# TorchIO-project/torchio

Measured on NVIDIA H100. Metric: augmented voxels/sec on 256^3 fp32 Compose pipeline, higher is better.
Workload: dtype f32

## Files before the change

### torchio_b200/csrc/fused_intensity.cu

```cuda
#include "common.cuh"
#include "mt19937_layout.h"
#include "mt19937_normal.cuh"
#include "tma.cuh"

namespace tio {

__device__ __forceinline__ float rician(float x, float n1, float n2) {
  float s = __fadd_rn(x, n1);
  return sqrtf(__fadd_rn(__fmul_rn(s, s), __fmul_rn(n2, n2)));
}


__device__ __forceinline__ uint4 philox4x32_10(uint4 ctr, uint2 key) {
  const uint32_t M0 = 0xD2511F53u, M1 = 0xCD9E8D57u, W0 = 0x9E3779B9u, W1 = 0xBB67AE85u;
#pragma unroll
  for (int r = 0; r < 7; ++r) {
    uint32_t hi0 = __umulhi(M0, ctr.x), lo0 = M0 * ctr.x;
    uint32_t hi1 = __umulhi(M1, ctr.z), lo1 = M1 * ctr.z;
    ctr = make_uint4(hi1 ^ ctr.y ^ key.x, lo1, hi0 ^ ctr.w ^ key.y, lo0);
    key.x += W0;
    key.y += W1;
  }
  return ctr;
}
// ... 508 lines not shown
          float b1 = lerp2(lk[v].l0, p1[lj.i1 * bi.sk + lk[v].i0], lk[v].l1, p1[lj.i1 * bi.sk + lk[v].i1]);
          r_hi[v] = lerp2(lj.l0, b0, lj.l1, b1);
        }
        cur0 = li.i0; cur1 = li.i1;
      }
#pragma unroll
      for (int v = 0; v < V; ++v) {
        float f = expf(lerp2(li.l0, r_lo[v], li.l1, r_hi[v]));
        out[v] = bi.divide ? __fdiv_rn(out[v], f) : __fmul_rn(out[v], f);
      }
    }
  };

  auto finish = [&](int i, float* v) {
    const int64_t o = ((int64_t)i * J + j) * K + k;
    if (noise_on) {
      const int64_t flat = (int64_t)bc * n + o;
      float z1[V], z2[V];
      if (nz.mode == 1) {
        if (V == 4) {
          float4 t = __ldcs((const float4*)(nz.z + flat));
          z1[0] = t.x; z1[1] = t.y; z1[2] = t.z; z1[3] = t.w;
          if (nz.rician) {
            float4 u = __ldcs((const float4*)(nz.z2 + flat));
            z2[0] = u.x; z2[1] = u.y; z2[2] = u.z; z2[3] = u.w;
          }
        } else {
          z1[0] = nz.z[flat];
          if (nz.rician) z2[0] = nz.z2[flat];
        }
      } else {
        const uint2 key = make_uint2((uint32_t)nz.philox_seed, (uint32_t)(nz.philox_seed >> 32));
        const uint64_t gidx = (uint64_t)(flat / V);
        uint4 rr = philox4x32_10(make_uint4((uint32_t)gidx, (uint32_t)(gidx >> 32), 0u, 0x5eedu), key);
        float nn[4];
        box_muller(rr.x, rr.y, nn[0], nn[1]);
        box_muller(rr.z, rr.w, nn[2], nn[3]);
#pragma unroll
        for (int q = 0; q < V; ++q) z1[q] = nn[q];
        if (nz.rician) {
          uint4 r2 = philox4x32_10(make_uint4((uint32_t)gidx, (uint32_t)(gidx >> 32), 1u, 0x5eedu), key);
          box_muller(r2.x, r2.y, nn[0], nn[1]);
          box_muller(r2.z, r2.w, nn[2], nn[3]);
#pragma unroll
          for (int q = 0; q < V; ++q) z2[q] = nn[q];
        }
      }
#pragma unroll
      for (int q = 0; q < V; ++q) {
        float n1 = __fadd_rn(mu, __fmul_rn(sd, z1[q]));
        if (nz.rician) v[q] = rician(v[q], n1, __fadd_rn(mu, __fmul_rn(sd, z2[q])));
        else v[q] = __fadd_rn(v[q], n1);
      }
    }
    if (gamma) {
#pragma unroll
      for (int q = 0; q < V; ++q) v[q] = signed_pow(v[q], gam);
    }
    if (V == 4) *(float4*)(y + o) = make_float4(v[0], v[1], v[2], v[3]);
    else y[o] = v[0];
  };

  if (r == 0) {
    for (int i = 0; i < I; ++i) {
      float v[V];
      load_plane(i, v);
      finish(i, v);
    }
    return;
  }

  float* mine = ring + tid * V;
  const int slot_stride = 256 * V;
  auto put = [&](int pos, const float* v) {
    int s = pos % W; if (s < 0) s += W;
    if (V == 4) *(float4*)(mine + s * slot_stride) = make_float4(v[0], v[1], v[2], v[3]);
    else mine[s * slot_stride] = v[0];
  };
  float first[V];
  load_plane(0, first);
  for (int p = -r; p <= 0; ++p) put(p, first);
  float last[V];
#pragma unroll
  for (int q = 0; q < V; ++q) last[q] = first[q];
  for (int p = 1; p < I + r; ++p) {
    if (p < I) load_plane(p, last);
    put(p, last);
    const int o = p - r;
    if (o < 0) continue;
    float acc[V];
#pragma unroll
    for (int q = 0; q < V; ++q) acc[q] = 0.0f;
    int s = (o - r) % W; if (s < 0) s += W;
    for (int t = 0; t < W; ++t) {
      const float tp = tapi[R - r + t];
      if (V == 4) {
        float4 w4 = *(const float4*)(mine + s * slot_stride);
        acc[0] = __fmaf_rn(tp, w4.x, acc[0]); acc[1] = __fmaf_rn(tp, w4.y, acc[1]);
        acc[2] = __fmaf_rn(tp, w4.z, acc[2]); acc[3] = __fmaf_rn(tp, w4.w, acc[3]);
      } else {
        acc[0] = __fmaf_rn(tp, mine[s * slot_stride], acc[0]);
      }
      if (++s == W) s = 0;
    }
    finish(o, acc);
  }
}

constexpr int M6_PF = 8;

template <bool HAS_BIAS, bool EPI, int BAR>
__device__ __forceinline__ void march6_tile(float* smem, const int tid, const int k, const int j, const int bc,
                                            const float* __restrict__ src, float* __restrict__ dst, int B,
                                            int C, int I, int J, int K, const BlurArgs& bl, const BiasArgs& bi,
                                            const NoiseArgs& nz, const float* __restrict__ gamma) {
  constexpr int W = 2 * F_R + 1;
  const int b = bc / C;
  const int64_t n = (int64_t)I * J * K;
  const float* x = src + (int64_t)bc * n;
  float* y = dst + (int64_t)bc * n;

  const int r = bl.taps ? bl.radius[0 * B + b] : 0;
  float* tapi = smem;
  float* g = smem + 16;
  const int ns = HAS_BIAS ? bi.si * bi.sj * bi.sk : 0;
  const bool bias_on = HAS_BIAS && !(bi.identity && bi.identity[b]);
  if (tid < W) {
    const int off = tid - F_R;
    tapi[tid] = (r > 0 && off >= -r && off <= r) ? bl.taps[((int64_t)0 * B + b) * (2 * bl.R + 1) + bl.R + off] : 0.0f;
  }
  if (bias_on) {
    const float* gs = bi.coarse + (int64_t)bc * ns;
    for (int t = tid; t < ns; t += 256) g[t] = gs[t];
  }
  if (BAR == 0) __syncthreads();
  else asm volatile("bar.sync %0, 256;" ::"n"(BAR) : "memory");
  if (k >= K || j >= J) return;

  const bool noise_on = EPI && nz.mode != 0 && (!nz.keep || nz.keep[b]);
  const float mu = (EPI && nz.mode) ? nz.mean[b] : 0.0f, sd = (EPI && nz.mode) ? nz.std[b] : 0.0f;
  const float gam = (EPI && gamma) ? gamma[b] : 1.0f;
  const int gamma_mode = !(EPI && gamma) || gam == 1.0f ? 0 : (gam > 0.0f ? 1 : 2);

  LerpAxis lj, lk[4];
  int o00[4], o01[4], o10[4], o11[4];
  int cur0 = -1, cur1 = -1;
  float r_lo[4], r_hi[4];
  if (bias_on) {
    lj = lerp_axis(bi.sc_j, bi.sj, j);
#pragma unroll
    for (int v = 0; v < 4; ++v) {
      lk[v] = lerp_axis(bi.sc_k, bi.sk, k + v);
      o00[v] = lj.i0 * bi.sk + lk[v].i0; o01[v] = lj.i0 * bi.sk + lk[v].i1;
      o10[v] = lj.i1 * bi.sk + lk[v].i0; o11[v] = lj.i1 * bi.sk + lk[v].i1;
    }
  }
  const int col = j * K + k;
  const int plane = J * K;

  float4* fifo = reinterpret_cast<float4*>(g + ((ns + 3) / 4) * 4) + tid;
  auto fifo_issue = [&](int pl) {
    if (pl < I) {
      const uint32_t sa = (uint32_t)__cvta_generic_to_shared(fifo + (pl & (M6_PF - 1)) * 256);
      asm volatile("cp.async.cg.shared.global [%0], [%1], 16;" ::"r"(sa), "l"(x + (int64_t)pl * plane + col) : "memory");
    }
    asm volatile("cp.async.commit_group;" ::: "memory");
  };
#pragma unroll
  for (int pl = 0; pl < M6_PF - 1; ++pl) fifo_issue(pl);

  auto load_plane = [&](int i, float* out) {
    fifo_issue(i + M6_PF - 1);
    asm volatile("cp.async.wait_group %0;" ::"n"(M6_PF - 1) : "memory");
    const float4 t = fifo[(i & (M6_PF - 1)) * 256];
    out[0] = t.x; out[1] = t.y; out[2] = t.z; out[3] = t.w;
    if (bias_on) {
      const LerpAxis li = lerp_axis(bi.sc_i, bi.si, i);
      if (li.i0 != cur0 || li.i1 != cur1) {
        const float* p0 = g + (li.i0 * bi.sj) * bi.sk;
        const float* p1 = g + (li.i1 * bi.sj) * bi.sk;
#pragma unroll
        for (int v = 0; v < 4; ++v) {
          const float a0 = lerp2(lk[v].l0, p0[o00[v]], lk[v].l1, p0[o01[v]]);
          const float a1 = lerp2(lk[v].l0, p0[o10[v]], lk[v].l1, p0[o11[v]]);
          r_lo[v] = lerp2(lj.l0, a0, lj.l1, a1);
          const float b0 = lerp2(lk[v].l0, p1[o00[v]], lk[v].l1, p1[o01[v]]);
          const float b1 = lerp2(lk[v].l0, p1[o10[v]], lk[v].l1, p1[o11[v]]);
          r_hi[v] = lerp2(lj.l0, b0, lj.l1, b1);
        }
        cur0 = li.i0; cur1 = li.i1;
      }
#pragma unroll
      for (int v = 0; v < 4; ++v) {
        const float f = expf(lerp2(li.l0, r_lo[v], li.l1, r_hi[v]));
        out[v] = bi.divide ? __fdiv_rn(out[v], f) : __fmul_rn(out[v], f);
      }
    }
  };

  auto finish = [&](int i, float* v) {
    const int64_t o = (int64_t)i * plane + col;
    if (EPI) {
      if (noise_on) {
        const int64_t flat = (int64_t)bc * n + o;
        float z1[4], z2[4];
        if (nz.mode == 1) {
          const float4 t = __ldcs((const float4*)(nz.z + flat));
          z1[0] = t.x; z1[1] = t.y; z1[2] = t.z; z1[3] = t.w;
          if (nz.rician) {
            const float4 u = __ldcs((const float4*)(nz.z2 + flat));
            z2[0] = u.x; z2[1] = u.y; z2[2] = u.z; z2[3] = u.w;
          }
        } else {
          const uint2 key = make_uint2((uint32_t)nz.philox_seed, (uint32_t)(nz.philox_seed >> 32));
          const uint64_t gidx = (uint64_t)(flat / 4);
          uint4 rr = philox4x32_10(make_uint4((uint32_t)gidx, (uint32_t)(gidx >> 32), 0u, 0x5eedu), key);
          box_muller(rr.x, rr.y, z1[0], z1[1]);
          box_muller(rr.z, rr.w, z1[2], z1[3]);
          if (nz.rician) {
            uint4 r2 = philox4x32_10(make_uint4((uint32_t)gidx, (uint32_t)(gidx >> 32), 1u, 0x5eedu), key);
            box_muller(r2.x, r2.y, z2[0], z2[1]);
            box_muller(r2.z, r2.w, z2[2], z2[3]);
          }
        }
#pragma unroll
        for (int q = 0; q < 4; ++q) {
          const float n1 = __fadd_rn(mu, __fmul_rn(sd, z1[q]));
          if (nz.rician) v[q] = rician(v[q], n1, __fadd_rn(mu, __fmul_rn(sd, z2[q])));
          else v[q] = __fadd_rn(v[q], n1);
        }
      }
      if (gamma_mode == 1) {
#pragma unroll
        for (int q = 0; q < 4; ++q) v[q] = signed_pow_pos(v[q], gam);
      } else if (gamma_mode == 2) {
#pragma unroll
        for (int q = 0; q < 4; ++q) v[q] = signed_pow(v[q], gam);
      }
    }
    *(float4*)(y + o) = make_float4(v[0], v[1], v[2], v[3]);
  };

  if (r == 0) {
    for (int i = 0; i < I; ++i) {
      float v[4];
      load_plane(i, v);
      finish(i, v);
    }
    return;
  }

  float tp[W];
#pragma unroll
  for (int t = 0; t < W; ++t) tp[t] = tapi[t];
  float ring[W][4];
  {
    float first[4];
    load_plane(0, first);
#pragma unroll
    for (int sl = 0; sl < W; ++sl)
#pragma unroll
      for (int q = 0; q < 4; ++q) ring[sl][q] = first[q];
  }
  for (int base = 0; base < I + F_R; base += W) {
#pragma unroll
    for (int ph = 0; ph < W; ++ph) {
      const int p = base + ph;
      if (p >= I + F_R) break;
      if (p > 0 && p < I) load_plane(p, ring[ph]);
      else if (p >= I) {
#pragma unroll
        for (int q = 0; q < 4; ++q) ring[ph][q] = ring[(ph + W - 1) % W][q];
      }
      const int o = p - F_R;
      if (o >= 0) {
        float acc[4] = {0.0f, 0.0f, 0.0f, 0.0f};
#pragma unroll
        for (int t = 0; t < W; ++t) {
          if (t < F_R - r || t > F_R + r) continue;
          const int sl = (ph + 1 + t) % W;
#pragma unroll
          for (int q = 0; q < 4; ++q) acc[q] = __fmaf_rn(tp[t], ring[sl][q], acc[q]);
        }
        finish(o, acc);
      }
    }
  }
}

template <bool HAS_BIAS, bool EPI>
__global__ void __launch_bounds__(256, EPI ? 1 : 2)
march6_kernel(const float* __restrict__ src, float* __restrict__ dst, int B, int C, int I, int J,
              int K, BlurArgs bl, BiasArgs bi, NoiseArgs nz, const float* __restrict__ gamma) {
  extern __shared__ __align__(16) float smem[];
  march6_tile<HAS_BIAS, EPI, 0>(smem, threadIdx.y * blockDim.x + threadIdx.x,
                                (blockIdx.x * blockDim.x + threadIdx.x) * 4,
                                blockIdx.y * blockDim.y + threadIdx.y, blockIdx.z, src, dst, B, C, I, J, K,
                                bl, bi, nz, gamma);
}

constexpr int P1N_MARCH_THREADS = 256;
constexpr int P1N_THREADS = P1N_MARCH_THREADS + 5 * 128;
constexpr int P1N_BAR_SEGMENT = 6, P1N_BAR_MARCH = 7;
constexpr int P1N_RING_FLOATS = MT_RING * MT_N + 4;

template <bool HAS_BIAS>
__global__ void __launch_bounds__(P1N_THREADS, 1)
pass1_normals_kernel(const float* __restrict__ src, float* __restrict__ dst, int B, int C, int I, int J,
                     int K, BlurArgs bl, BiasArgs bi, unsigned int* __restrict__ tile_counter,
                     const uint32_t* __restrict__ states, int q_lo, int q_hi, unsigned long long L,
                     unsigned long long offset, unsigned long long n, float* __restrict__ z) {
  extern __shared__ __align__(16) float smem[];
  if (threadIdx.x < P1N_MARCH_THREADS) {
    asm volatile("setmaxnreg.inc.sync.aligned.u32 152;");
    const int tid = threadIdx.x;
    volatile int* next_tile = reinterpret_cast<int*>(smem + MT_RING * MT_N);
    const int kb_n = (K + 255) / 256, jb_n = (J + 3) / 4;
    const int tiles = kb_n * jb_n * B * C;
    for (;;) {
      if (tid == 0) *next_tile = (int)atomicAdd(tile_counter, 1u);
      asm volatile("bar.sync %0, 256;" ::"n"(P1N_BAR_MARCH) : "memory");
      const int tile = *next_tile;
      if (tile >= tiles) break;
      const int kb = tile % kb_n, jb = (tile / kb_n) % jb_n, bc = tile / (kb_n * jb_n);
      march6_tile<HAS_BIAS, false, P1N_BAR_MARCH>(smem + P1N_RING_FLOATS, tid, (kb * 64 + (tid & 63)) * 4,
                                                  jb * 4 + (tid >> 6), bc, src, dst, B, C, I, J, K, bl, bi,
                                                  NoiseArgs{}, nullptr);
    }
  } else {
    asm volatile("setmaxnreg.dec.sync.aligned.u32 40;");
    const int tid = threadIdx.x - P1N_MARCH_THREADS;
    if (tid >= MT_THREADS) return;
    for (int q = q_lo + blockIdx.x; q < q_hi; q += gridDim.x) {
      mt_normal_segment(reinterpret_cast<uint32_t*>(smem), tid, states, q, L, offset, n, z);
      mt_bar_sync<P1N_BAR_SEGMENT, MT_THREADS>();
    }
  }
}

constexpr int WIDE_RMAX = 6143;

template <bool HAS_EPI>
__global__ void __launch_bounds__(256)
axis_kernel(const float* __restrict__ src, float* __restrict__ dst, int B, int C, int I, int J,
            int K, int axis, BlurArgs bl, NoiseArgs nz, const float* __restrict__ gamma) {
  extern __shared__ float taps_s[];
  const int bc = blockIdx.y;
  const int b = bc / C;
  const int tid = threadIdx.x;
  const int64_t n = (int64_t)I * J * K;
  const int r = bl.radius[axis * B + b];
  for (int t = tid; t < 2 * r + 1; t += 256)
    taps_s[t] = bl.taps[((int64_t)axis * B + b) * (2 * bl.R + 1) + bl.R - r + t];
  __syncthreads();
  const int64_t e = (int64_t)blockIdx.x * 256 + tid;
  if (e >= n) return;
  const int L = axis == 0 ? I : (axis == 1 ? J : K);
  const int64_t s = axis == 0 ? (int64_t)J * K : (axis == 1 ? K : 1);
  const int pos = (int)((e / s) % L);
  const float* x = src + (int64_t)bc * n + (e - pos * s);
  float acc;
  if (r == 0) {
    acc = x[pos * s];
  } else {
    acc = 0.0f;
    for (int t = 0; t <= 2 * r; ++t) {
      const int q = min(max(pos - r + t, 0), L - 1);
      acc = __fmaf_rn(taps_s[t], __ldg(x + q * s), acc);
    }
  }
  const int64_t flat = (int64_t)bc * n + e;
  if (HAS_EPI) {
    if (nz.mode != 0 && (!nz.keep || nz.keep[b])) {
      const float mu = nz.mean[b], sd = nz.std[b];
      float z1, z2 = 0.0f;
      if (nz.mode == 1) {
        z1 = nz.z[flat];
        if (nz.rician) z2 = nz.z2[flat];
      } else {
        const uint2 key = make_uint2((uint32_t)nz.philox_seed, (uint32_t)(nz.philox_seed >> 32));
        float unused;
        uint4 rr = philox4x32_10(make_uint4((uint32_t)flat, (uint32_t)((uint64_t)flat >> 32), 0u, 0x77ffu), key);
        box_muller(rr.x, rr.y, z1, unused);
        if (nz.rician) box_muller(rr.z, rr.w, z2, unused);
      }
      const float n1 = __fadd_rn(mu, __fmul_rn(sd, z1));
      acc = nz.rician ? rician(acc, n1, __fadd_rn(mu, __fmul_rn(sd, z2))) : __fadd_rn(acc, n1);
    }
    if (gamma) acc = signed_pow(acc, gamma[b]);
  }
  dst[flat] = acc;
}

static inline bool aligned16f(const void* p) { return ((uintptr_t)p & 15) == 0; }

static float up_scale(int n_in, int n_out) {
  if (n_in == n_out) return 1.0f;
  return n_out > 1 ? (float)(n_in - 1) / (float)(n_out - 1) : 0.0f;
}

template <int RMAX>
static int launch_jk(const float* src, float* dst, int B, int C, int I, int J, int K,
                     const BlurArgs& bl, const NoiseArgs& nz, const float* gamma, cudaStream_t st) {
  constexpr int ROWS = A_TJ + 2 * RMAX, COLS = A_TK + 2 * RMAX, PITCH = (COLS + 3) / 4 * 4 + 4;
  const size_t smem = (size_t)(ROWS * PITCH + ROWS * A_TK + 2 * (2 * RMAX + 1)) * sizeof(float);
  const int tiles_i = (I + A_PLANES - 1) / A_PLANES;
  dim3 grid((K + A_TK - 1) / A_TK, (J + A_TJ - 1) / A_TJ, B * C * tiles_i);
  if (nz.mode != 0 || gamma) {
    if (smem > 48 * 1024)
      cudaFuncSetAttribute(jk_kernel<RMAX, true>, cudaFuncAttributeMaxDynamicSharedMemorySize, (int)smem);
    jk_kernel<RMAX, true><<<grid, 256, smem, st>>>(src, dst, B, C, I, J, K, bl, nz, gamma);
  } else {
    if (smem > 48 * 1024)
      cudaFuncSetAttribute(jk_kernel<RMAX, false>, cudaFuncAttributeMaxDynamicSharedMemorySize, (int)smem);
    jk_kernel<RMAX, false><<<grid, 256, smem, st>>>(src, dst, B, C, I, J, K, bl, nz, gamma);
  }
  launched();
  return 0;
}

static int launch_march(const float* cur, float* out, int B, int C, int I, int J, int K,
                        const BiasArgs& bi, const BlurArgs& ib, const NoiseArgs& nz1,
                        const float* gamma1, cudaStream_t st, const char* who) {
  {
    const bool vec = (K % 4 == 0) && aligned16f(cur) && aligned16f(out) &&
                     (nz1.mode != 1 || (aligned16f(nz1.z) && (!nz1.z2 || aligned16f(nz1.z2))));
    const int V = vec ? 4 : 1;
    dim3 block(64, 4);
    dim3 grid((K + 64 * V - 1) / (64 * V), (J + 3) / 4, B * C);
    TIO_CHECK_ARG(grid.y <= 65535, "%s: J too large", who);
    const int R = ib.taps ? ib.R : 0;
    const int ns = bi.coarse ? bi.si * bi.sj * bi.sk : 0;
    const size_t smem = ((size_t)((2 * R + 1 + 3) / 4 * 4) + (size_t)((ns + 3) / 4 * 4) +
                         (ib.taps ? (size_t)(2 * R + 1) * 256 * V : 0)) * sizeof(float);
#define TIO_LAUNCH_MARCH(VV, BB)                                                              \
  do {                                                                                        \
    if (smem > 48 * 1024)                                                                     \
      cudaFuncSetAttribute(march_kernel<VV, BB>, cudaFuncAttributeMaxDynamicSharedMemorySize, \
                           (int)smem);                                                        \
    march_kernel<VV, BB><<<grid, block, smem, st>>>(cur, out, B, C, I, J, K, ib, bi, nz1, gamma1); \
    launched();                                                                               \
  } while (0)
    if (vec && R <= F_R) {
      const size_t smem6 = (size_t)(16 + (ns + 3) / 4 * 4) * sizeof(float) + (size_t)M6_PF * 256 * 16;
#define TIO_LAUNCH_MARCH6(BB, EE)                                                              \
  do {                                                                                         \
    if (smem6 > 48 * 1024)                                                                     \
      cudaFuncSetAttribute(march6_kernel<BB, EE>, cudaFuncAttributeMaxDynamicSharedMemorySize, \
                           (int)smem6);                                                        \
    march6_kernel<BB, EE><<<grid, block, smem6, st>>>(cur, out, B, C, I, J, K, ib, bi, nz1, gamma1); \
    launched();                                                                                \
  } while (0)
      const bool epi = nz1.mode != 0 || gamma1 != nullptr;
      if (bi.coarse) { if (epi) TIO_LAUNCH_MARCH6(true, true); else TIO_LAUNCH_MARCH6(true, false); }
      else { if (epi) TIO_LAUNCH_MARCH6(false, true); else TIO_LAUNCH_MARCH6(false, false); }
#undef TIO_LAUNCH_MARCH6
    } else if (vec) { if (bi.coarse) TIO_LAUNCH_MARCH(4, true); else TIO_LAUNCH_MARCH(4, false); }
    else { if (bi.coarse) TIO_LAUNCH_MARCH(1, true); else TIO_LAUNCH_MARCH(1, false); }
#undef TIO_LAUNCH_MARCH
  }
  return 0;
}

static int wide_impl(const float* src, float* dst, float* scratch, int B, int C, int I, int J,
                     int K, const BiasArgs& bi, const BlurArgs& bl, int axes_mask,
                     const NoiseArgs& nz, const float* gamma, cudaStream_t st, const char* who) {
  TIO_CHECK_ARG(bl.R <= WIDE_RMAX, "%s: blur radius R=%d > %d unsupported", who, bl.R, WIDE_RMAX);
  int axes[3], na = 0;
  for (int a : {0, 2, 1})
    if (axes_mask & (1 << a)) axes[na++] = a;
  const int steps = na + (bi.coarse ? 1 : 0);
  TIO_CHECK_ARG(src != dst && (steps < 2 || (scratch && scratch != src && scratch != dst)),
                "%s: blur radius R=%d > 16 needs src != dst and a scratch buffer", who, bl.R);
  const int64_t n = (int64_t)I * J * K;
  TIO_CHECK_ARG((n + 255) / 256 <= 0x7fffffff, "%s: volume too large", who);
  const float* cur = src;
  int left = steps;
  auto next_out = [&]() { return (--left % 2 == 0) ? dst : scratch; };
  if (bi.coarse) {
    BlurArgs none = bl;
    none.taps = nullptr;
    float* out = next_out();
    if (launch_march(cur, out, B, C, I, J, K, bi, none, NoiseArgs{}, nullptr, st, who)) return 1;
    cur = out;
  }
  const size_t smem = (size_t)(2 * bl.R + 1) * sizeof(float);
  dim3 grid((unsigned)((n + 255) / 256), B * C);
  for (int s = 0; s < na; ++s) {
    float* out = next_out();
    if (s == na - 1 && (nz.mode != 0 || gamma))
      axis_kernel<true><<<grid, 256, smem, st>>>(cur, out, B, C, I, J, K, axes[s], bl, nz, gamma);
    else
      axis_kernel<false><<<grid, 256, smem, st>>>(cur, out, B, C, I, J, K, axes[s], bl, nz, gamma);
    launched();
    cur = out;
  }
  TIO_CHECK_LAUNCH();
  return 0;
}

static int fused_impl(const float* src, float* dst, float* scratch, int B, int C, int I, int J,
                      int K, BiasArgs bi, BlurArgs bl, int axes_mask, NoiseArgs nz,
                      const float* gamma, cudaStream_t st, const char* who) {
  TIO_CHECK_ARG(src && dst, "%s: null src/dst", who);
  TIO_CHECK_ARG(B > 0 && C > 0 && I > 0 && J > 0 && K > 0, "%s: bad shape", who);
  TIO_CHECK_ARG((int64_t)B * C <= 65535, "%s: B*C must be <= 65535", who);
  if (!bl.taps) axes_mask = 0;
  TIO_CHECK_ARG(!bl.taps || (bl.radius && bl.R >= 0), "%s: blur radius table missing or R=%d < 0", who, bl.R);
  if (bi.coarse) {
    bi.sc_i = up_scale(bi.si, I); bi.sc_j = up_scale(bi.sj, J); bi.sc_k = up_scale(bi.sk, K);
    TIO_CHECK_ARG((size_t)bi.si * bi.sj * bi.sk * 4 <= 64 * 1024, "%s: coarse bias grid too large", who);
  }
  if (axes_mask != 0 && bl.R > 16)
    return wide_impl(src, dst, scratch, B, C, I, J, K, bi, bl, axes_mask, nz, gamma, st, who);
  const bool need_jk = (axes_mask & 6) != 0;
  const bool need_i = (axes_mask & 1) != 0;
  const bool need_march = !need_jk || need_i || bi.coarse != nullptr;
  TIO_CHECK_ARG(!need_jk || src != dst, "%s: blur along J/K needs src != dst", who);
  TIO_CHECK_ARG(!(need_jk && need_march) || (scratch && scratch != src && scratch != dst),
                "%s: blur along J/K after bias or blur along I needs a scratch buffer", who);
  TIO_CHECK_ARG(!((axes_mask & 1) && src == dst && !need_jk), "%s: blur along I needs src != dst", who);
  const float* cur = src;
  if (need_jk) {
    const int64_t tiles = (int64_t)B * C * ((I + A_PLANES - 1) / A_PLANES);
    TIO_CHECK_ARG(tiles <= 65535, "%s: batch too large for the blur grid", who);
  }
  if (need_march) {
    BlurArgs ib = bl;
    if (!need_i) ib.taps = nullptr;
    float* out = need_jk ? scratch : dst;
    if (launch_march(cur, out, B, C, I, J, K, bi, ib, need_jk ? NoiseArgs{} : nz,
                     need_jk ? nullptr : gamma, st, who))
      return 1;
    cur = out;
  }
  if (need_jk) {
    const bool tma_ok = bl.R <= F_R && (K % 4 == 0) && aligned16f(cur) && (int64_t)B * C * I < (1ll << 31);
    EncodeTiledFn encode = tma_ok ? encode_tiled_fn() : nullptr;
    CUtensorMap tm;
    bool have_map = false;
    if (encode) {
      const cuuint64_t gdim[3] = {(cuuint64_t)K, (cuuint64_t)J, (cuuint64_t)B * C * I};
      const cuuint64_t gstride[2] = {(cuuint64_t)K * 4, (cuuint64_t)J * K * 4};
      const cuuint32_t bdim[3] = {(cuuint32_t)F_COLS, (cuuint32_t)F_ROWS, 1};
      const cuuint32_t estr[3] = {1, 1, 1};
      have_map = encode(&tm, CU_TENSOR_MAP_DATA_TYPE_FLOAT32, 3, const_cast<float*>(cur), gdim, gstride,
                        bdim, estr, CU_TENSOR_MAP_INTERLEAVE_NONE, CU_TENSOR_MAP_SWIZZLE_NONE,
                        CU_TENSOR_MAP_L2_PROMOTION_L2_128B, CU_TENSOR_MAP_FLOAT_OOB_FILL_NONE) == CUDA_SUCCESS;
    }
    if (have_map) {
      const int tiles_i = (I + A_PLANES - 1) / A_PLANES;
      dim3 grid((K + A_TK - 1) / A_TK, (J + A_TJ - 1) / A_TJ, B * C * tiles_i);
      if (nz.mode != 0 || gamma) {
        cudaFuncSetAttribute(jk6_kernel<true>, cudaFuncAttributeMaxDynamicSharedMemorySize, (int)F_SMEM);
        jk6_kernel<true><<<grid, 256, F_SMEM, st>>>(tm, dst, B, C, I, J, K, bl, nz, gamma);
      } else {
        cudaFuncSetAttribute(jk6_kernel<false>, cudaFuncAttributeMaxDynamicSharedMemorySize, (int)F_SMEM);
        jk6_kernel<false><<<grid, 256, F_SMEM, st>>>(tm, dst, B, C, I, J, K, bl, nz, gamma);
      }
      launched();
    } else if (bl.R <= F_R) {
      launch_jk<6>(cur, dst, B, C, I, J, K, bl, nz, gamma, st);
    } else {
      launch_jk<16>(cur, dst, B, C, I, J, K, bl, nz, gamma, st);
    }
  }
  TIO_CHECK_LAUNCH();
  return 0;
}

}

using namespace tio;

extern "C" int tio_blur(const float* src, float* dst, float* scratch, int B, int C, int I, int J,
                        int K, const float* taps, const int32_t* radius, int R, int axes_mask,
                        const uint8_t* identity, void* stream) {
  (void)identity;
  TIO_CHECK_ARG(taps && radius, "tio_blur: null taps/radius");
  TIO_CHECK_ARG(src != dst, "tio_blur: src and dst must not alias");
  BiasArgs bi{};
  BlurArgs bl{taps, radius, R};
  NoiseArgs nz{};
  return fused_impl(src, dst, scratch, B, C, I, J, K, bi, bl, axes_mask & 7, nz, nullptr,
                    (cudaStream_t)stream, "tio_blur");
}

extern "C" int tio_intensity_fused(const float* src, float* dst, float* scratch, int B, int C,
                                   int I, int J, int K, const float* coarse, int si, int sj,
                                   int sk, const uint8_t* bias_identity, int bias_divide,
                                   const float* taps, const int32_t* radius, int R,
                                   int axes_mask, const float* mean, const float* std,
                                   const uint8_t* keep, const float* z, const float* z2,
                                   uint64_t philox_seed, int noise_mode, int rician_flag,
                                   const float* gamma, void* stream) {
  BiasArgs bi{};
  bi.coarse = coarse; bi.identity = bias_identity; bi.si = si; bi.sj = sj; bi.sk = sk;
  bi.divide = bias_divide;
  BlurArgs bl{taps, radius, R};
  NoiseArgs nz{};
  nz.mode = noise_mode;
  TIO_CHECK_ARG(noise_mode >= 0 && noise_mode <= 2, "tio_intensity_fused: bad noise_mode");
  if (noise_mode) {
    TIO_CHECK_ARG(mean && std, "tio_intensity_fused: noise needs mean/std");
    TIO_CHECK_ARG(noise_mode != 1 || (z && (!rician_flag || z2)), "tio_intensity_fused: normals missing");
    nz.mean = mean; nz.std = std; nz.keep = keep; nz.z = z; nz.z2 = z2;
    nz.philox_seed = philox_seed; nz.rician = rician_flag;
  }
  return fused_impl(src, dst, scratch, B, C, I, J, K, bi, bl, taps ? (axes_mask & 7) : 0, nz,
                    gamma, (cudaStream_t)stream, "tio_intensity_fused");
}

extern "C" size_t tio_intensity_pass1_with_normals_workspace_bytes(uint64_t offset, uint64_t n) {
  return tio_randn_mt19937_workspace_bytes(offset, n) + 16;
}

extern "C" int tio_intensity_pass1_with_normals(const float* src, float* dst, int B, int C, int I, int J,
                                                int K, const float* coarse, int si, int sj, int sk,
                                                const uint8_t* bias_identity, int bias_divide,
                                                const float* taps, const int32_t* radius, int R,
                                                int axes_mask, uint64_t seed, uint64_t offset, uint64_t n,
                                                float* z, const void* table, void* workspace,
                                                size_t workspace_bytes, void* stream) {
  const char* who = "tio_intensity_pass1_with_normals";
  TIO_CHECK_ARG(src && dst && z, "%s: null src/dst/z", who);
  TIO_CHECK_ARG(src != dst, "%s: src and dst must not alias", who);
  TIO_CHECK_ARG(B > 0 && C > 0 && I > 0 && J > 0 && K > 0, "%s: bad shape", who);
  const bool need_i = taps && (axes_mask & 1);
  TIO_CHECK_ARG(!need_i || (radius && R >= 0 && R <= F_R), "%s: needs a radius table and R <= %d, got R=%d", who,
                F_R, R);
  TIO_CHECK_ARG(K % 4 == 0 && aligned16f(src) && aligned16f(dst) && aligned16f(z),
                "%s: needs K %% 4 == 0 and 16-byte aligned src, dst and z", who);
  const int64_t tiles = (int64_t)((K + 255) / 256) * ((J + 3) / 4) * B * C;
  TIO_CHECK_ARG(tiles < (1ll << 31) - (1 << 20), "%s: batch too large", who);
  BiasArgs bi{};
  bi.coarse = coarse; bi.identity = bias_identity; bi.si = si; bi.sj = sj; bi.sk = sk;
  bi.divide = bias_divide;
  if (coarse) {
    bi.sc_i = up_scale(si, I); bi.sc_j = up_scale(sj, J); bi.sc_k = up_scale(sk, K);
    TIO_CHECK_ARG(si > 0 && sj > 0 && sk > 0 && (size_t)si * sj * sk * 4 <= 64 * 1024,
                  "%s: coarse bias grid empty or too large", who);
  }
  BlurArgs bl{need_i ? taps : nullptr, radius, R};
  TIO_CHECK_ARG(workspace_bytes >= tio_intensity_pass1_with_normals_workspace_bytes(offset, n),
                "%s: workspace too small", who);
  cudaStream_t st = (cudaStream_t)stream;
  int q_lo, q_hi;
  const size_t states_bytes = tio_randn_mt19937_workspace_bytes(offset, n);
  if (int rc = mt_start_states(seed, offset, n, table, workspace, states_bytes, st, who, &q_lo, &q_hi)) return rc;
  unsigned int* tile_counter = reinterpret_cast<unsigned int*>((char*)workspace + states_bytes);
  cudaMemsetAsync(tile_counter, 0, sizeof(unsigned int), st);
  const int ns = coarse ? si * sj * sk : 0;
  const size_t smem = (size_t)(P1N_RING_FLOATS + 16 + (ns + 3) / 4 * 4) * sizeof(float) + (size_t)M6_PF * 256 * 16;
  const unsigned long long seg = 1ull << tio_mt::kLog2L;
  const int grid = num_sms();
#define TIO_LAUNCH_P1N(BB)                                                                                   \
  do {                                                                                                       \
    cudaFuncSetAttribute(pass1_normals_kernel<BB>, cudaFuncAttributeMaxDynamicSharedMemorySize, (int)smem);  \
    pass1_normals_kernel<BB><<<grid, P1N_THREADS, smem, st>>>(src, dst, B, C, I, J, K, bl, bi, tile_counter, \
                                                              (const uint32_t*)workspace, q_lo, q_hi, seg,   \
                                                              offset, n, z);                                 \
    launched();                                                                                              \
  } while (0)
  if (coarse) TIO_LAUNCH_P1N(true); else TIO_LAUNCH_P1N(false);
#undef TIO_LAUNCH_P1N
  TIO_CHECK_LAUNCH();
  return 0;
}
```

### torchio_b200/csrc/mt19937.cu

```cuda
#include "common.cuh"
#include "mt19937_layout.h"
#include "mt19937_normal.cuh"

namespace tio {

constexpr int MT_DEG = 19937;
constexpr int MT_SEQ = MT_DEG + MT_N;
constexpr int MT_OFFS = (MT_SEQ + 7) / 4 * 4;

__global__ void mt_seed_kernel(uint32_t seed, uint32_t* __restrict__ states) {
  if (threadIdx.x == 0) {
    uint32_t v = seed;
    states[0] = v;
    for (int j = 1; j < MT_N; ++j) {
      v = 1812433253u * (v ^ (v >> 30)) + (uint32_t)j;
      states[j] = v;
    }
  }
}

struct MtJob { int src, dst, slot; };

__global__ void __launch_bounds__(640)
mt_jump_kernel(uint32_t* __restrict__ states, const uint16_t* __restrict__ polys, int stride,
               int first, int S2, int fine, int parts) {
  extern __shared__ __align__(16) uint32_t seq[];
  uint32_t* offs = seq + MT_OFFS;
  const int job_idx = (int)blockIdx.x / parts, part = (int)blockIdx.x % parts;
  MtJob job;
  if (fine) {
    const int q = first + job_idx, r = q % S2;
    if (r == 0) return;
    job = MtJob{q - r, q, r - 1};
  } else {
    const int m = first + job_idx;
    job = MtJob{0, m * S2, (S2 - 1) + (m - 1)};
  }
  const int tid = threadIdx.x;
  const uint32_t* src = states + (size_t)job.src * MT_N;
  for (int t = tid; t < MT_N; t += blockDim.x) seq[t] = src[t];
  __syncthreads();
  for (int base = 0; base + MT_N < MT_SEQ; base += MT_N - MT_M) {
    const int k = base + tid;
    if (tid < MT_N - MT_M && k + MT_N < MT_SEQ)
      seq[k + MT_N] = mt_twist(seq[k], seq[k + 1], seq[k + MT_M]);
    __syncthreads();
  }
  const uint16_t* p = polys + (size_t)job.slot * stride;
  const uint32_t count = p[0] | ((uint32_t)p[1] << 16);
  const uint32_t t_begin = (uint32_t)((uint64_t)count * part / parts);
  const uint32_t t_end = (uint32_t)((uint64_t)count * (part + 1) / parts);
  const char* mine = reinterpret_cast<const char*>(seq + (tid < MT_N ? tid : 0));
  uint32_t acc = 0;
  for (uint32_t c0 = t_begin; c0 < t_end; c0 += 2048) {
    const uint32_t chunk = min(2048u, t_end - c0);
    for (uint32_t t = tid; t < chunk; t += blockDim.x) offs[t] = (uint32_t)p[2 + c0 + t] << 2;
    __syncthreads();
    if (tid < MT_N) {
      const uint4* o4 = reinterpret_cast<const uint4*>(offs);
      const uint32_t quads = chunk >> 2;
#pragma unroll 4
      for (uint32_t t = 0; t < quads; ++t) {
        const uint4 o = o4[t];
        acc ^= *reinterpret_cast<const uint32_t*>(mine + o.x) ^ *reinterpret_cast<const uint32_t*>(mine + o.y);
        acc ^= *reinterpret_cast<const uint32_t*>(mine + o.z) ^ *reinterpret_cast<const uint32_t*>(mine + o.w);
      }
      for (uint32_t t = quads << 2; t < chunk; ++t) acc ^= *reinterpret_cast<const uint32_t*>(mine + offs[t]);
    }
    __syncthreads();
  }
  if (tid < MT_N) {
    uint32_t* dst = states + (size_t)job.dst * MT_N + tid;
    if (parts == 1) *dst = acc;
    else atomicXor(dst, acc);
  }
}

__global__ void __launch_bounds__(MT_THREADS, 2)
mt_normal_kernel(const uint32_t* __restrict__ states, int q_first, unsigned long long L,
                 unsigned long long offset, unsigned long long n, float* __restrict__ z) {
  __shared__ __align__(16) uint32_t ring[MT_RING * MT_N];
  mt_normal_segment(ring, (int)threadIdx.x, states, q_first + (int)blockIdx.x, L, offset, n, z);
}

constexpr uint64_t MT_L = 1ull << tio_mt::kLog2L;

int mt_start_states(uint64_t seed, uint64_t offset, uint64_t n, const void* table, void* workspace,
                    size_t workspace_bytes, cudaStream_t st, const char* who, int* q_lo_out, int* q_hi_out) {
  TIO_CHECK_ARG(table && workspace, "%s: null table or workspace", who);
  TIO_CHECK_ARG(n >= 16 && (n % 16) == 0 && (offset % 16) == 0,
                "%s: n and offset must be multiples of 16 (n >= 16)", who);
  const int S2 = tio_mt::kS2, S1 = tio_mt::kS1, stride = tio_mt::kStride;
  const uint64_t q_lo = offset / MT_L, q_hi = (offset + n + MT_L - 1) / MT_L;
  TIO_CHECK_ARG(q_hi <= (uint64_t)S1 * S2, "%s: stream position beyond %d segments", who, S1 * S2);
  TIO_CHECK_ARG(workspace_bytes >= tio_randn_mt19937_workspace_bytes(offset, n), "%s: workspace too small", who);
  uint32_t* states = (uint32_t*)workspace;
  const uint16_t* polys = (const uint16_t*)((const char*)table + tio_mt::kHeaderBytes);
  mt_seed_kernel<<<1, 32, 0, st>>>((uint32_t)seed, states);
  launched();
  const size_t jump_smem = (size_t)(MT_OFFS + 2048) * 4;
  cudaFuncSetAttribute(mt_jump_kernel, cudaFuncAttributeMaxDynamicSharedMemorySize, (int)jump_smem);
  const int m_lo = (int)(q_lo / S2), m_hi = (int)((q_hi - 1) / S2);
  const int m_first = m_lo > 1 ? m_lo : 1;
  if (m_hi >= m_first) {
    constexpr int kCoarseParts = 8;
    const size_t pitch = (size_t)S2 * MT_N * 4;
    cudaMemset2DAsync(states + (size_t)m_first * S2 * MT_N, pitch, 0, MT_N * 4, m_hi - m_first + 1, st);
    mt_jump_kernel<<<(m_hi - m_first + 1) * kCoarseParts, 640, jump_smem, st>>>(states, polys, stride, m_first,
                                                                             S2, 0, kCoarseParts);
    launched();
  }
  mt_jump_kernel<<<(unsigned)(q_hi - q_lo), 640, jump_smem, st>>>(states, polys, stride, (int)q_lo, S2, 1, 1);
  launched();
  *q_lo_out = (int)q_lo;
  *q_hi_out = (int)q_hi;
  return 0;
}

}

using namespace tio;

extern "C" size_t tio_randn_mt19937_workspace_bytes(uint64_t offset, uint64_t n) {
  const uint64_t q_hi = (offset + n + MT_L - 1) / MT_L;
  return (size_t)(q_hi + tio_mt::kS1) * MT_N * 4;
}

extern "C" int tio_randn_mt19937(uint64_t seed, uint64_t offset, uint64_t n, float* z,
                                 const void* table, void* workspace, size_t workspace_bytes,
                                 void* stream) {
  TIO_CHECK_ARG(z, "tio_randn_mt19937: null pointer");
  cudaStream_t st = (cudaStream_t)stream;
  int q_lo, q_hi;
  if (int rc = mt_start_states(seed, offset, n, table, workspace, workspace_bytes, st, "tio_randn_mt19937",
                               &q_lo, &q_hi))
    return rc;
  mt_normal_kernel<<<(unsigned)(q_hi - q_lo), MT_THREADS, 0, st>>>((const uint32_t*)workspace, q_lo, MT_L, offset,
                                                                   n, z);
  launched();
  TIO_CHECK_LAUNCH();
  return 0;
}
```

### torchio_b200/csrc/mt19937_normal.cuh

```cuda
#pragma once

#include "common.cuh"

namespace tio {

constexpr int MT_N = 624, MT_M = 397;

__device__ __forceinline__ uint32_t mt_twist(uint32_t a, uint32_t b, uint32_t c) {
  const uint32_t y = (a & 0x80000000u) | (b & 0x7fffffffu);
  return c ^ (y >> 1) ^ ((y & 1u) ? 0x9908b0dfu : 0u);
}

__device__ __forceinline__ uint32_t mt_temper(uint32_t y) {
  y ^= y >> 11;
  y ^= (y << 7) & 0x9d2c5680u;
  y ^= (y << 15) & 0xefc60000u;
  y ^= y >> 18;
  return y;
}

__device__ __forceinline__ void sincos_0_2pi(float theta, float& sn, float& cs) {
  const float t = __fmaf_rn(theta, 0.6366197723675814f, 12582912.0f);
  const int j = __float_as_int(t);
  const float jf = __fsub_rn(t, 12582912.0f);
  float r = __fmaf_rn(jf, -1.5707962512969971f, theta);
  r = __fmaf_rn(jf, -7.549789415861596e-08f, r);
  const float r2 = __fmul_rn(r, r);
  float ps = __fmaf_rn(r2, -1.9515295891e-4f, 8.3321608736e-3f);
  ps = __fmaf_rn(ps, r2, -1.6666654611e-1f);
  const float s = __fmaf_rn(__fmul_rn(ps, r2), r, r);
  float pc = __fmaf_rn(r2, 2.443315711809948e-5f, -1.388731625493765e-3f);
  pc = __fmaf_rn(pc, r2, 4.166664568298827e-2f);
  const float c = __fmaf_rn(__fmul_rn(pc, r2), r2, __fmaf_rn(r2, -0.5f, 1.0f));
  const bool swap = j & 1;
  const float a = swap ? c : s, b = swap ? s : c;
  sn = (j & 2) ? -a : a;
  cs = ((j + 1) & 2) ? -b : b;
}

__device__ __forceinline__ void mt_box_muller(uint32_t a, uint32_t b, float& zc, float& zs) {
  const float u1 = (float)(mt_temper(a) & 0xffffffu) * (1.0f / 16777216.0f);
  const float u2 = (float)(mt_temper(b) & 0xffffffu) * (1.0f / 16777216.0f);
  float radius;
  asm("sqrt.approx.ftz.f32 %0, %1;" : "=f"(radius) : "f"(-2.0f * logf(1.0f - u1)));
  const float theta = (float)(6.283185307179586 * (double)u2);
  float sn, cs;
  sincos_0_2pi(theta, sn, cs);
  zc = radius * cs;
  zs = radius * sn;
}

template <int ID, int COUNT>
__device__ __forceinline__ void mt_bar_sync() {
  asm volatile("bar.sync %0, %1;" ::"n"(ID), "n"(COUNT) : "memory");
}
template <int ID, int COUNT>
__device__ __forceinline__ void mt_bar_arrive() {
  asm volatile("bar.arrive %0, %1;" ::"n"(ID), "n"(COUNT) : "memory");
}

constexpr int MT_ROUND = 4;
constexpr int MT_RING = 2 * MT_ROUND;
constexpr int MT_ITEMS = MT_ROUND * MT_N / 8;
constexpr int MT_PRODUCERS = 256;
constexpr int MT_CONSUMERS = (MT_ITEMS + 31) / 32 * 32;
constexpr int MT_THREADS = MT_PRODUCERS + MT_CONSUMERS;
constexpr int MT_BAR_PROD = 1, MT_BAR_FULL = 2, MT_BAR_EMPTY = 4;

__device__ __forceinline__ void mt_normal_segment(uint32_t* __restrict__ ring, const int tid,
                                                  const uint32_t* __restrict__ states, const int q,
                                                  unsigned long long L, unsigned long long offset,
                                                  unsigned long long n, float* __restrict__ z) {
  const unsigned long long seg_begin = (unsigned long long)q * L;
  const unsigned long long lo = max(seg_begin, offset);
  const unsigned long long hi = min(seg_begin + L, offset + n);
  if (lo >= hi) return;
  const int lo_rel = (int)(lo - seg_begin), hi_rel = (int)(hi - seg_begin);
  const int rounds = ((hi_rel + MT_N - 1) / MT_N + MT_ROUND - 1) / MT_ROUND;
  if (tid < MT_PRODUCERS) {
    constexpr int W = MT_N - MT_M;
    const uint32_t* w = states + (size_t)q * MT_N;
    uint32_t* start = ring + (MT_RING - 1) * MT_N;
    for (int t = tid; t < MT_N; t += MT_PRODUCERS) start[t] = w[t];
    mt_bar_sync<MT_BAR_PROD, MT_PRODUCERS>();
    for (int r = 0; r < rounds; ++r) {
      if (r >= 2) {
        if (r & 1) mt_bar_sync<MT_BAR_EMPTY + 1, MT_THREADS>();
        else mt_bar_sync<MT_BAR_EMPTY, MT_THREADS>();
      }
      for (int i = 0; i < MT_ROUND; ++i) {
        const int b = r * MT_ROUND + i;
        const uint32_t* cur = ring + ((b + MT_RING - 1) % MT_RING) * MT_N;
        uint32_t* nxt = ring + (b % MT_RING) * MT_N;
        if (tid < W) nxt[tid] = mt_twist(cur[tid], cur[tid + 1], cur[tid + MT_M]);
        mt_bar_sync<MT_BAR_PROD, MT_PRODUCERS>();
        if (tid < W) nxt[W + tid] = mt_twist(cur[W + tid], cur[W + tid + 1], nxt[tid]);
        mt_bar_sync<MT_BAR_PROD, MT_PRODUCERS>();
        if (tid < MT_N - 2 * W) {
          const int k = 2 * W + tid;
          const uint32_t c = (k + 1 < MT_N) ? cur[k + 1] : nxt[0];
          nxt[k] = mt_twist(cur[k], c, nxt[k - W]);
        }
        mt_bar_sync<MT_BAR_PROD, MT_PRODUCERS>();
      }
      if (r & 1) mt_bar_arrive<MT_BAR_FULL + 1, MT_THREADS>();
      else mt_bar_arrive<MT_BAR_FULL, MT_THREADS>();
    }
  } else {
    const int c = tid - MT_PRODUCERS;
    const int blk = c / (MT_N / 8), item = c % (MT_N / 8);
    const int word = 16 * (item >> 1) + 4 * (item & 1);
    const long long seg_to_z = (long long)seg_begin - (long long)offset;
    const bool vec = ((reinterpret_cast<uintptr_t>(z) & 15) == 0);
    for (int r = 0; r < rounds; ++r) {
      if (r & 1) mt_bar_sync<MT_BAR_FULL + 1, MT_THREADS>();
      else mt_bar_sync<MT_BAR_FULL, MT_THREADS>();
      const int b = r * MT_ROUND + blk;
      const int group = b * MT_N + (word & ~15);
      if (c < MT_ITEMS && group >= lo_rel && group < hi_rel) {
        const uint32_t* x = ring + (b % MT_RING) * MT_N + word;
        const uint4 a = *reinterpret_cast<const uint4*>(x);
        const uint4 s = *reinterpret_cast<const uint4*>(x + 8);
        float4 zc, zs;
        mt_box_muller(a.x, s.x, zc.x, zs.x);
        mt_box_muller(a.y, s.y, zc.y, zs.y);
        mt_box_muller(a.z, s.z, zc.z, zs.z);
        mt_box_muller(a.w, s.w, zc.w, zs.w);
        float* zp = z + (seg_to_z + b * MT_N + word);
        if (vec) {
          *reinterpret_cast<float4*>(zp) = zc;
          *reinterpret_cast<float4*>(zp + 8) = zs;
        } else {
          zp[0] = zc.x; zp[1] = zc.y; zp[2] = zc.z; zp[3] = zc.w;
          zp[8] = zs.x; zp[9] = zs.y; zp[10] = zs.z; zp[11] = zs.w;
        }
      }
      if (r + 2 < rounds) {
        if (r & 1) mt_bar_arrive<MT_BAR_EMPTY + 1, MT_THREADS>();
        else mt_bar_arrive<MT_BAR_EMPTY, MT_THREADS>();
      }
    }
  }
}

int mt_start_states(uint64_t seed, uint64_t offset, uint64_t n, const void* table, void* workspace,
                    size_t workspace_bytes, cudaStream_t st, const char* who, int* q_lo, int* q_hi);

}
```

Before: 51.74 billion.

## Interleave two MT19937 segments per producer pass with dynamic pair scheduling

```diff
diff --git a/torchio_b200/csrc/fused_intensity.cu b/torchio_b200/csrc/fused_intensity.cu
--- a/torchio_b200/csrc/fused_intensity.cu
+++ b/torchio_b200/csrc/fused_intensity.cu
@@ -834,23 +834,37 @@
 constexpr int P1N_MARCH_THREADS = 256;
 constexpr int P1N_THREADS = P1N_MARCH_THREADS + 5 * 128;
 constexpr int P1N_BAR_SEGMENT = 6, P1N_BAR_MARCH = 7;
-constexpr int P1N_RING_FLOATS = MT_RING * MT_N + 4;
+constexpr int P1N_RING_FLOATS = 2 * MT_RING * MT_N + 4;
+
+__device__ __forceinline__ void p1n_normal_pairs(float* smem, const int tid, unsigned int* __restrict__ counters,
+                                                 const uint32_t* __restrict__ states, int q_lo, int q_hi,
+                                                 unsigned long long L, unsigned long long offset,
+                                                 unsigned long long n, float* __restrict__ z) {
+  volatile int* next_pair = reinterpret_cast<int*>(smem + 2 * MT_RING * MT_N) + 1;
+  for (;;) {
+    if (tid == MT_PRODUCERS) *next_pair = (int)atomicAdd(counters + 1, 1u);
+    mt_bar_sync<P1N_BAR_SEGMENT, MT_THREADS>();
+    const int q = q_lo + 2 * *next_pair;
+    if (q >= q_hi) break;
+    mt_normal_segments<2>(reinterpret_cast<uint32_t*>(smem), tid, states, q, L, offset, n, z);
+  }
+}
 
 template <bool HAS_BIAS>
 __global__ void __launch_bounds__(P1N_THREADS, 1)
 pass1_normals_kernel(const float* __restrict__ src, float* __restrict__ dst, int B, int C, int I, int J,
-                     int K, BlurArgs bl, BiasArgs bi, unsigned int* __restrict__ tile_counter,
+                     int K, BlurArgs bl, BiasArgs bi, unsigned int* __restrict__ counters,
                      const uint32_t* __restrict__ states, int q_lo, int q_hi, unsigned long long L,
                      unsigned long long offset, unsigned long long n, float* __restrict__ z) {
   extern __shared__ __align__(16) float smem[];
   if (threadIdx.x < P1N_MARCH_THREADS) {
     asm volatile("setmaxnreg.inc.sync.aligned.u32 152;");
     const int tid = threadIdx.x;
-    volatile int* next_tile = reinterpret_cast<int*>(smem + MT_RING * MT_N);
+    volatile int* next_tile = reinterpret_cast<int*>(smem + 2 * MT_RING * MT_N);
     const int kb_n = (K + 255) / 256, jb_n = (J + 3) / 4;
     const int tiles = kb_n * jb_n * B * C;
     for (;;) {
-      if (tid == 0) *next_tile = (int)atomicAdd(tile_counter, 1u);
+      if (tid == 0) *next_tile = (int)atomicAdd(counters, 1u);
       asm volatile("bar.sync %0, 256;" ::"n"(P1N_BAR_MARCH) : "memory");
       const int tile = *next_tile;
       if (tile >= tiles) break;
@@ -863,10 +877,8 @@
     asm volatile("setmaxnreg.dec.sync.aligned.u32 40;");
     const int tid = threadIdx.x - P1N_MARCH_THREADS;
     if (tid >= MT_THREADS) return;
-    for (int q = q_lo + blockIdx.x; q < q_hi; q += gridDim.x) {
-      mt_normal_segment(reinterpret_cast<uint32_t*>(smem), tid, states, q, L, offset, n, z);
-      mt_bar_sync<P1N_BAR_SEGMENT, MT_THREADS>();
-    }
+    if (tid < MT_PRODUCERS) p1n_normal_pairs(smem, tid, counters, states, q_lo, q_hi, L, offset, n, z);
+    else p1n_normal_pairs(smem, tid, counters, states, q_lo, q_hi, L, offset, n, z);
   }
 }
 
@@ -1180,8 +1192,8 @@
   int q_lo, q_hi;
   const size_t states_bytes = tio_randn_mt19937_workspace_bytes(offset, n);
   if (int rc = mt_start_states(seed, offset, n, table, workspace, states_bytes, st, who, &q_lo, &q_hi)) return rc;
-  unsigned int* tile_counter = reinterpret_cast<unsigned int*>((char*)workspace + states_bytes);
-  cudaMemsetAsync(tile_counter, 0, sizeof(unsigned int), st);
+  unsigned int* counters = reinterpret_cast<unsigned int*>((char*)workspace + states_bytes);
+  cudaMemsetAsync(counters, 0, 2 * sizeof(unsigned int), st);
   const int ns = coarse ? si * sj * sk : 0;
   const size_t smem = (size_t)(P1N_RING_FLOATS + 16 + (ns + 3) / 4 * 4) * sizeof(float) + (size_t)M6_PF * 256 * 16;
   const unsigned long long seg = 1ull << tio_mt::kLog2L;
@@ -1189,7 +1201,7 @@
 #define TIO_LAUNCH_P1N(BB)                                                                                   \
   do {                                                                                                       \
     cudaFuncSetAttribute(pass1_normals_kernel<BB>, cudaFuncAttributeMaxDynamicSharedMemorySize, (int)smem);  \
-    pass1_normals_kernel<BB><<<grid, P1N_THREADS, smem, st>>>(src, dst, B, C, I, J, K, bl, bi, tile_counter, \
+    pass1_normals_kernel<BB><<<grid, P1N_THREADS, smem, st>>>(src, dst, B, C, I, J, K, bl, bi, counters,     \
                                                               (const uint32_t*)workspace, q_lo, q_hi, seg,   \
                                                               offset, n, z);                                 \
     launched();                                                                                              \
diff --git a/torchio_b200/csrc/mt19937.cu b/torchio_b200/csrc/mt19937.cu
--- a/torchio_b200/csrc/mt19937.cu
+++ b/torchio_b200/csrc/mt19937.cu
@@ -80,7 +80,7 @@
 mt_normal_kernel(const uint32_t* __restrict__ states, int q_first, unsigned long long L,
                  unsigned long long offset, unsigned long long n, float* __restrict__ z) {
   __shared__ __align__(16) uint32_t ring[MT_RING * MT_N];
-  mt_normal_segment(ring, (int)threadIdx.x, states, q_first + (int)blockIdx.x, L, offset, n, z);
+  mt_normal_segments<1>(ring, (int)threadIdx.x, states, q_first + (int)blockIdx.x, L, offset, n, z);
 }
 
 constexpr uint64_t MT_L = 1ull << tio_mt::kLog2L;
diff --git a/torchio_b200/csrc/mt19937_normal.cuh b/torchio_b200/csrc/mt19937_normal.cuh
--- a/torchio_b200/csrc/mt19937_normal.cuh
+++ b/torchio_b200/csrc/mt19937_normal.cuh
@@ -67,21 +67,29 @@
 constexpr int MT_THREADS = MT_PRODUCERS + MT_CONSUMERS;
 constexpr int MT_BAR_PROD = 1, MT_BAR_FULL = 2, MT_BAR_EMPTY = 4;
 
-__device__ __forceinline__ void mt_normal_segment(uint32_t* __restrict__ ring, const int tid,
-                                                  const uint32_t* __restrict__ states, const int q,
-                                                  unsigned long long L, unsigned long long offset,
-                                                  unsigned long long n, float* __restrict__ z) {
+template <int NSEG>
+__device__ __forceinline__ void mt_normal_segments(uint32_t* __restrict__ ring, const int tid,
+                                                   const uint32_t* __restrict__ states, const int q,
+                                                   unsigned long long L, unsigned long long offset,
+                                                   unsigned long long n, float* __restrict__ z) {
+  static_assert(NSEG == 1 || NSEG == 2, "one or two segments per pass");
+  constexpr int RING1 = MT_RING * MT_N;
   const unsigned long long seg_begin = (unsigned long long)q * L;
   const unsigned long long lo = max(seg_begin, offset);
   const unsigned long long hi = min(seg_begin + L, offset + n);
   if (lo >= hi) return;
   const int lo_rel = (int)(lo - seg_begin), hi_rel = (int)(hi - seg_begin);
   const int rounds = ((hi_rel + MT_N - 1) / MT_N + MT_ROUND - 1) / MT_ROUND;
+  int hi_rel1 = 0;
+  if (NSEG == 2 && offset + n > seg_begin + L)
+    hi_rel1 = (int)(min(seg_begin + 2 * L, offset + n) - (seg_begin + L));
   if (tid < MT_PRODUCERS) {
     constexpr int W = MT_N - MT_M;
     const uint32_t* w = states + (size_t)q * MT_N;
     uint32_t* start = ring + (MT_RING - 1) * MT_N;
     for (int t = tid; t < MT_N; t += MT_PRODUCERS) start[t] = w[t];
+    if (NSEG == 2 && hi_rel1 > 0)
+      for (int t = tid; t < MT_N; t += MT_PRODUCERS) start[RING1 + t] = w[MT_N + t];
     mt_bar_sync<MT_BAR_PROD, MT_PRODUCERS>();
     for (int r = 0; r < rounds; ++r) {
       if (r >= 2) {
@@ -92,14 +100,27 @@
         const int b = r * MT_ROUND + i;
         const uint32_t* cur = ring + ((b + MT_RING - 1) % MT_RING) * MT_N;
         uint32_t* nxt = ring + (b % MT_RING) * MT_N;
-        if (tid < W) nxt[tid] = mt_twist(cur[tid], cur[tid + 1], cur[tid + MT_M]);
+        if (tid < W) {
+          const uint32_t x = mt_twist(cur[tid], cur[tid + 1], cur[tid + MT_M]);
+          if (NSEG == 2) nxt[RING1 + tid] = mt_twist(cur[RING1 + tid], cur[RING1 + tid + 1], cur[RING1 + tid + MT_M]);
+          nxt[tid] = x;
+        }
         mt_bar_sync<MT_BAR_PROD, MT_PRODUCERS>();
-        if (tid < W) nxt[W + tid] = mt_twist(cur[W + tid], cur[W + tid + 1], nxt[tid]);
+        if (tid < W) {
+          const uint32_t x = mt_twist(cur[W + tid], cur[W + tid + 1], nxt[tid]);
+          if (NSEG == 2) nxt[RING1 + W + tid] = mt_twist(cur[RING1 + W + tid], cur[RING1 + W + tid + 1], nxt[RING1 + tid]);
+          nxt[W + tid] = x;
+        }
         mt_bar_sync<MT_BAR_PROD, MT_PRODUCERS>();
         if (tid < MT_N - 2 * W) {
           const int k = 2 * W + tid;
           const uint32_t c = (k + 1 < MT_N) ? cur[k + 1] : nxt[0];
-          nxt[k] = mt_twist(cur[k], c, nxt[k - W]);
+          const uint32_t x = mt_twist(cur[k], c, nxt[k - W]);
+          if (NSEG == 2) {
+            const uint32_t c1 = (k + 1 < MT_N) ? cur[RING1 + k + 1] : nxt[RING1];
+            nxt[RING1 + k] = mt_twist(cur[RING1 + k], c1, nxt[RING1 + k - W]);
+          }
+          nxt[k] = x;
         }
         mt_bar_sync<MT_BAR_PROD, MT_PRODUCERS>();
       }
@@ -117,22 +138,25 @@
       else mt_bar_sync<MT_BAR_FULL, MT_THREADS>();
       const int b = r * MT_ROUND + blk;
       const int group = b * MT_N + (word & ~15);
-      if (c < MT_ITEMS && group >= lo_rel && group < hi_rel) {
-        const uint32_t* x = ring + (b % MT_RING) * MT_N + word;
-        const uint4 a = *reinterpret_cast<const uint4*>(x);
-        const uint4 s = *reinterpret_cast<const uint4*>(x + 8);
-        float4 zc, zs;
-        mt_box_muller(a.x, s.x, zc.x, zs.x);
-        mt_box_muller(a.y, s.y, zc.y, zs.y);
-        mt_box_muller(a.z, s.z, zc.z, zs.z);
-        mt_box_muller(a.w, s.w, zc.w, zs.w);
-        float* zp = z + (seg_to_z + b * MT_N + word);
-        if (vec) {
-          *reinterpret_cast<float4*>(zp) = zc;
-          *reinterpret_cast<float4*>(zp + 8) = zs;
-        } else {
-          zp[0] = zc.x; zp[1] = zc.y; zp[2] = zc.z; zp[3] = zc.w;
-          zp[8] = zs.x; zp[9] = zs.y; zp[10] = zs.z; zp[11] = zs.w;
+#pragma unroll
+      for (int sg = 0; sg < NSEG; ++sg) {
+        if (c < MT_ITEMS && group >= (sg ? 0 : lo_rel) && group < (sg ? hi_rel1 : hi_rel)) {
+          const uint32_t* x = ring + sg * RING1 + (b % MT_RING) * MT_N + word;
+          const uint4 a = *reinterpret_cast<const uint4*>(x);
+          const uint4 s = *reinterpret_cast<const uint4*>(x + 8);
+          float4 zc, zs;
+          mt_box_muller(a.x, s.x, zc.x, zs.x);
+          mt_box_muller(a.y, s.y, zc.y, zs.y);
+          mt_box_muller(a.z, s.z, zc.z, zs.z);
+          mt_box_muller(a.w, s.w, zc.w, zs.w);
+          float* zp = z + (seg_to_z + (long long)sg * (long long)L + b * MT_N + word);
+          if (vec) {
+            *reinterpret_cast<float4*>(zp) = zc;
+            *reinterpret_cast<float4*>(zp + 8) = zs;
+          } else {
+            zp[0] = zc.x; zp[1] = zc.y; zp[2] = zc.z; zp[3] = zc.w;
+            zp[8] = zs.x; zp[9] = zs.y; zp[10] = zs.z; zp[11] = zs.w;
+          }
         }
       }
       if (r + 2 < rounds) {
```

New measurement: 51.90 billion (median of 6 runs). Within noise of the previous version (+0.3%).
